# SeanNaren/deepspeech.pytorch

Hardware: NVIDIA H100
Metric: utterances/sec (train step, 161x1000 spectrogram) (higher is better)
Workload: dtype fp16-operands(rnn)+tf32(conv/fc)

## Files before the change

deepspeech.pytorch_b200/csrc/rnn_persistent_tc.cu:

```cuda
#include <cooperative_groups.h>
#include <cuda_fp16.h>
#include <dlfcn.h>
#include <stdlib.h>

#include "common.cuh"
#include "rnn_cells.cuh"
#include "rnn_common.cuh"
#include "tc_common.cuh"

namespace cg = cooperative_groups;

namespace ds2 {

namespace rp {
constexpr int UT = 16;
constexpr int MM = 64;
constexpr int BK = 32;
constexpr int STAGES = 8;
constexpr int THREADS = 288;
constexpr int A_BYTES = MM * 128;
constexpr long long SPIN_LIMIT = 4000000000LL;
}

struct PersistParams {
// ... 475 lines not shown
  int max_clusters = 0;
  if (cudaOccupancyMaxActiveClusters(&max_clusters, kern, &c.cfg) != cudaSuccess) {
    (void)cudaGetLastError();
    return -1;
  }
  return max_clusters * cluster;
}

template <typename Prepare>
static int launch_sweep(SweepKernel kern, int cluster, int per_dir, size_t smem, int fit, bool per_dir_ok,
                        size_t ctl_bytes, const char* what, const char* fallback, PersistParams& p, cudaStream_t st,
                        Prepare&& prepare) {
  int grid = p.D * per_dir, launches = 1;
  if (fit < grid) {
    if (!per_dir_ok || fit < per_dir) return 1;
    grid = per_dir;
    launches = p.D;
  }
  if (int rc = prepare()) return rc;
  DS2_CHECK_CUDA(cudaMemsetAsync(p.err, 0, ctl_bytes, st));
  SweepConfig c(cluster, grid, smem, st);
  for (int li = 0; li < launches; ++li) {
    p.d0 = li;
    if (cluster == 0) {
      void* args[] = {&p};
      DS2_CHECK_CUDA(cudaLaunchCooperativeKernel((const void*)kern, dim3(grid), dim3(rp::THREADS), args, smem, st));
    } else {
      const cudaError_t le = cudaLaunchKernelEx(&c.cfg, kern, p);
      if (le != cudaSuccess) {
        (void)cudaGetLastError();
        if (li == 0) {
          if (fallback)
            fprintf(stderr, "ds2_b200: WARNING %s launch failed (%s); using %s\n", what, cudaGetErrorString(le), fallback);
          return 1;
        }
        set_error("%s: second launch failed: %s", what, cudaGetErrorString(le));
        return DS2_ERR_CUDA;
      }
    }
    g_launches.fetch_add(1, std::memory_order_relaxed);
  }
  DS2_LAUNCH(sweep_check_kernel, 1, 1, 0, st, p.err);
  return DS2_OK;
}

static size_t fwd_smem_bytes(int NB) {
  using namespace rp;
  size_t NBp = NB + 1;
  return 1024 + (size_t)STAGES * (A_BYTES + (size_t)NB * 128) + (5 * UT * NBp + NB + 4) * sizeof(float) +
         (2 * STAGES + 2) * sizeof(uint64_t) + 64 + tc::acc_image_bytes(NB);
}

static size_t splitk_res_ws_bytes(int G, int T, int B, int H, int D);

size_t rnn_sweep_tc_workspace_bytes(int rnn, int T, int B, int H, int D) {
  const int G = rnn == DS2_RNN_LSTM ? 4 : (rnn == DS2_RNN_GRU ? 3 : 1);
  const size_t fwd = 4096 + align_up((size_t)D * G * H * H * 2, 256) + align_up((size_t)D * T * B * H * 2, 256);
  const size_t bwd = splitk_res_ws_bytes(G, T, B, H, D);
  return (fwd > bwd ? fwd : bwd) + 256;
}

static bool fwd_eligible(const SeqArgs& a) {
  if (a.h0 || a.c0) return false;
  if (a.H % 32 != 0 || a.B > 256 || a.T < 2) return false;
  return vec_ok(a.gates, a.hseq, a.aux);
}

__global__ void f32_to_f16_kernel(size_t n, const float* __restrict__ in, __half* __restrict__ out) {
  size_t i = (size_t)blockIdx.x * blockDim.x + threadIdx.x, stride = (size_t)gridDim.x * blockDim.x;
  for (; i < n; i += stride) out[i] = __float2half_rn(in[i]);
}

static size_t res_smem_bytes(int NB, int H) {
  using namespace rp;
  size_t NBp = NB + 1;
  return 1024 + (size_t)(H / 64) * (A_BYTES + (size_t)NB * 128) + (5 * UT * NBp + NB + 4) * sizeof(float) +
         (32 + STAGES + 2) * sizeof(uint64_t) + 64 + tc::acc_image_bytes(NB);
}

static size_t res_ws_bytes(int G, int T, int B, int H, int D) {
  return 4096 + align_up((size_t)D * G * H * H * 2, 256) + align_up((size_t)D * T * B * H * 2, 256);
}

static int f16_weight_maps(const SeqArgs& a, PersistParams& p, void* ws, int chunks, cudaStream_t st) {
  using namespace rp;
  const int G = a.G;
  __half* w16 = reinterpret_cast<__half*>(static_cast<char*>(ws) + 4096);
  p.h16 = reinterpret_cast<__half*>(static_cast<char*>(ws) + 4096 + align_up((size_t)a.D * G * a.H * a.H * 2, 256));
  const size_t wn = (size_t)G * a.H * a.H;
  p.box3 = chunks % 4 == 0;
  for (int d = 0; d < a.D; ++d) {
    DS2_LAUNCH(f32_to_f16_kernel, 132 * 4, 256, 0, st, wn, a.w_hh[d], w16 + (size_t)d * wn);
    int rc = make_tmap_f16(&p.tmW[d], w16 + (size_t)d * wn, 3, a.H, a.H, G, (size_t)a.H, (size_t)a.H * a.H, 64, UT, G);
    if (rc) return rc;
    rc = make_tmap_f16(&p.tmV[d], p.h16 + (size_t)d * a.T * a.B * a.H, 2, a.H, a.T * a.B, 1, (size_t)a.H, 0, 64, a.B, 1);
    if (rc) return rc;
    if (p.box3) {
      rc = make_tmap_f16(&p.tmV3[d], p.h16 + (size_t)d * a.T * a.B * a.H, 3, 64, a.T * a.B, a.H / 64, (size_t)a.H, 64, 64,
                         p.NB, 4);
      if (rc) return rc;
    }
  }
  return DS2_OK;
}

template <int RNN>
static int launch_fwd_resident(const SeqArgs& a, void* ws, size_t ws_bytes, cudaStream_t st) {
  const int G = RNN == DS2_RNN_LSTM ? 4 : (RNN == DS2_RNN_GRU ? 3 : 1);
  if (a.H % 64 != 0 || a.H / 64 > 32) return 1;
  if (!vec_ok(a.gates, a.hseq, a.aux)) return 1;
  if (ws_bytes < res_ws_bytes(G, a.T, a.B, a.H, a.D)) return 1;
  PersistParams p = sweep_params(a, rp::UT, "DS2_TRACE_FWD", ws);
  if (p.NB > 128) return 1;
  const size_t smem = one_cta_per_sm(res_smem_bytes(p.NB, a.H));
  if (smem > 227 * 1024) return 1;
  const SweepKernel kern = rnn_fwd_persist_kernel<RNN, true>;
  static DeviceOnce attr_once;
  int fit = 0;
  if (int rc = opt_in_smem(attr_once, {kern})) return rc;
  if (int rc = coop_fit(kern, smem, &fit)) return rc;
  return launch_sweep(kern, 0, p.NT, smem, fit, true, 4096, nullptr, nullptr, p, st,
                      [&] { return f16_weight_maps(a, p, ws, a.H / 64, st); });
}

template <int RNN>
static int launch_fwd_splitk(const SeqArgs& a, void* ws, size_t ws_bytes, cudaStream_t st);

template <int RNN>
static int launch_fwd(const SeqArgs& a, void* ws, size_t ws_bytes, cudaStream_t st) {
  using namespace rp;
  const int G = RNN == DS2_RNN_LSTM ? 4 : (RNN == DS2_RNN_GRU ? 3 : 1);
  if (!getenv("DS2_NO_RESIDENT")) {
    if (RNN != DS2_RNN_TANH && env_flag("DS2_FWD_SPLITK", 1)) {
      constexpr int R = RNN == DS2_RNN_TANH ? DS2_RNN_LSTM : RNN;
      int rc = launch_fwd_splitk<R>(a, ws, ws_bytes, st);
      if (rc != 1) return rc;
    }
    int rc = launch_fwd_resident<RNN>(a, ws, ws_bytes, st);
    if (rc != 1) return rc;
  }
  PersistParams p = sweep_params(a, UT, "DS2_TRACE_FWD", ws);
  if (p.NB > 128) return 1;
  if (ws_bytes < 4096) return 1;
  const size_t smem = one_cta_per_sm(fwd_smem_bytes(p.NB));
  if (smem > 227 * 1024) return 1;
  const SweepKernel kern = rnn_fwd_persist_kernel<RNN, false>;
  static DeviceOnce attr_once;
  int fit = 0;
  if (int rc = opt_in_smem(attr_once, {kern})) return rc;
  if (int rc = coop_fit(kern, smem, &fit)) return rc;
  return launch_sweep(kern, 0, p.NT, smem, fit, true, 4096, nullptr, nullptr, p, st, [&] {
    for (int d = 0; d < a.D; ++d) {
      int rc = make_tmap_3d(&p.tmW[d], a.w_hh[d], a.H, a.H, G, (size_t)a.H, (size_t)a.H * a.H, BK, UT, G);
      if (rc) return rc;
      rc = make_tmap_2d(&p.tmV[d], a.hseq + (size_t)d * a.T * a.B * a.H, a.T * a.B, a.H, a.H, a.B, BK);
      if (rc) return rc;
    }
    return 0;
  });
}

int rnn_sweep_fwd_tc(int rnn, const SeqArgs& a, void* ws, size_t ws_bytes, cudaStream_t st) {
  if (!fwd_eligible(a)) return 1;
  if (rnn == DS2_RNN_LSTM) return launch_fwd<DS2_RNN_LSTM>(a, ws, ws_bytes, st);
  if (rnn == DS2_RNN_GRU) return launch_fwd<DS2_RNN_GRU>(a, ws, ws_bytes, st);
  return launch_fwd<DS2_RNN_TANH>(a, ws, ws_bytes, st);
}

template <int RNN>
__global__ void __launch_bounds__(rp::THREADS, 1) rnn_bwd_persist_kernel(const __grid_constant__ PersistParams p) {
  using namespace rp;
  using namespace tc;
  constexpr int G = RNN == DS2_RNN_LSTM ? 4 : (RNN == DS2_RNN_GRU ? 3 : 1);
  extern __shared__ uint8_t smem_raw[];
  uint8_t* smem = smem_raw + ((1024u - (tc::smem_u32(smem_raw) & 1023u)) & 1023u);
  const int NB = p.NB, B = p.B, T = p.T, H = p.H, D = p.D;
// ... 607 lines not shown
            __half h[NPF];
#pragma unroll
            for (int j = 0; j < NPF; ++j) {
              h[j] = to_half_sat(o[g][j] * nscale);
              t16[((size_t)g * H + j) * TBs] = h[j];
            }
            const __half2 lo = __halves2half2(h[0], h[1]), hi = __halves2half2(h[2], h[3]);
            uint2 pk;
            pk.x = *reinterpret_cast<const unsigned int*>(&lo);
            pk.y = *reinterpret_cast<const unsigned int*>(&hi);
            *reinterpret_cast<uint2*>(r16 + g * H) = pk;
          }
          if (RNN == DS2_RNN_GRU) {
            __half* a16 = p.auxn16T + ((size_t)d * H + u0 + uq) * TBs + col;
#pragma unroll
            for (int j = 0; j < NPF; ++j) a16[(size_t)j * TBs] = to_half_sat(o[4][j] * nscale);
          }
        }
      };
      const bool defer = RES && p.defer && single;
      float sv[5][NPF];
      if (single) {
        finish4(b_own, kc, pdy, pvalid, sv);
        if (!defer && b_own < B) store_dg(b_own, sv);
      } else {
        for (int b = b_own; b < B; b += 32) {
          load_coefs(b, kc, pdy, pvalid);
          finish4(b, kc, pdy, pvalid, sv);
          store_dg(b, sv);
        }
      }
      if (RES) {
#pragma unroll
        for (int o = 16; o > 0; o >>= 1) lmax = fmaxf(lmax, __shfl_xor_sync(0xffffffffu, lmax, o));
        if (lane == 0) atomicMax(cta_max, __float_as_uint(lmax));
      }
      if (e == 0) trace_stamp(p.trace, p.T, step, 8);
      named_bar_sync(1, 128);
      if (e == 0) {
        trace_stamp(p.trace, p.T, step, 9);
        if (RES) {
          atomicMax(p.gmax + (size_t)d * (T + 1) + step + 1, cta_max[0]);
          cta_max[0] = 0u;
        }
        fence_proxy_async_global();
        trace_stamp(p.trace, p.T, step, 10);
        red_release(ctr, 1u);
        trace_stamp(p.trace, p.T, step, 11);
        trace_stamp_ns(p.trace, p.T, step, 12);
      }
      if (defer) {
        if (b_own < B) store_dg(b_own, sv);
        if (e == 0) trace_stamp(p.trace, p.T, step, 13);
      }
    }
    if (p.dbias[d]) {
      named_bar_sync(1, 128);
      float* red = part;
#pragma unroll
      for (int i = 0; i < 5; ++i) {
#pragma unroll
        for (int j = 0; j < 4; ++j) {
          float v = bsum[i][j];
          v += __shfl_xor_sync(0xffffffffu, v, 4);
          v += __shfl_xor_sync(0xffffffffu, v, 8);
          v += __shfl_xor_sync(0xffffffffu, v, 16);
          if (lane < 4) red[(q * 5 + i) * 16 + 4 * lane + j] = v;
        }
      }
      named_bar_sync(1, 128);
      if (e < 80) {
        const int i = e / 16, u = e % 16;
        const float v = (red[(0 * 5 + i) * 16 + u] + red[(1 * 5 + i) * 16 + u]) +
                        (red[(2 * 5 + i) * 16 + u] + red[(3 * 5 + i) * 16 + u]);
        if (i < G) p.dbias[d][(size_t)i * H + u0 + u] = v;
        else if (RNN == DS2_RNN_GRU && i == 4) p.dbias_hn[d][u0 + u] = v;
      }
    }
  }
  __syncthreads();
  if constexpr (!XG) cluster_sync_all();
}

template <int RNN, int NKR_T = 0>
__global__ void __launch_bounds__(rp::THREADS, 1) rnn_fwd_splitk_kernel(const __grid_constant__ PersistParams p) {
  using namespace rp;
  using namespace tc;
  constexpr int G = RNN == DS2_RNN_LSTM ? 4 : 3;
  constexpr int AW = 128 * 128;
  extern __shared__ uint8_t smem_raw[];
  uint8_t* smem = smem_raw + ((1024u - (tc::smem_u32(smem_raw) & 1023u)) & 1023u);
  const int NB = p.NB, B = p.B, T = p.T, H = p.H, D = p.D;
  const int B_BYTES = NB * 128;
  const int NBp = NB + 1;
  const int NKR = NKR_T ? NKR_T : H / 128;
  const int NG = grp_count(NKR);
  float* part = reinterpret_cast<float*>(smem + NKR * (AW + B_BYTES));
  float* cst = part + 2 * xt_slice(64, NB);
  int* lens_s = reinterpret_cast<int*>(cst + UT * NBp);
  uint64_t* full = reinterpret_cast<uint64_t*>(lens_s + ((NB + 1) & ~1));
  uint64_t* wbar = full + 8;
  uint64_t* accum_bar = wbar + 1;
  uint64_t* part_bar = accum_bar + 1;
  float* acc_img = reinterpret_cast<float*>(part_bar + 1);

  const int warp = threadIdx.x / 32, lane = threadIdx.x % 32;
  const int rank = blockIdx.x & 1, cl = blockIdx.x >> 1;
  const int NTc = H / 32;
  const int d = p.d0 + cl / NTc, U0 = (cl % NTc) * 32;
  const int u0 = U0 + rank * UT;
  const int GH = G * H;
  unsigned int* ctr = p.bar + 32 * d;
  const unsigned int n_arrive = (unsigned int)(NTc * 2);

  if (warp == 0 && lane == 0) {
    tma_prefetch_desc(&p.tmW[d]);
    tma_prefetch_desc(&p.tmV[d]);
    for (int i = 0; i < 8; ++i) mbar_init(&full[i], 1);
    mbar_init(wbar, 1);
    mbar_init(accum_bar, 1);
    mbar_init(part_bar, 1);
    fence_barrier_init();
  }
  for (int i = threadIdx.x; i < UT * NBp; i += THREADS) cst[i] = 0.f;
  for (int i = threadIdx.x; i < NB; i += THREADS) lens_s[i] = i < B ? p.len[i] : 0;
  __syncthreads();
  cluster_sync_all();
  const int kc0 = rank * NKR;

  if (warp == 8) {
    if (lane == 0) {
      mbar_arrive_expect_tx(wbar, (uint32_t)(NKR * 2 * G * UT * 128));
      for (int c = 0; c < NKR; ++c) {
        tma_load_3d(smem + c * AW, &p.tmW[d], wbar, (kc0 + c) * 64, U0, 0);
        tma_load_3d(smem + c * AW + 64 * 128, &p.tmW[d], wbar, (kc0 + c) * 64, U0 + UT, 0);
      }
      uint8_t* hbuf = smem + NKR * AW;
      for (int step = 1; step < T; ++step) {
        const int t = d == 0 ? step : T - 1 - step;
        const int tp = d == 0 ? t - 1 : t + 1;
        grid_wait_counter(ctr, n_arrive * (unsigned int)step, p.err);
        fence_proxy_async_global();
        trace_stamp(p.trace, p.T, step, 0);
        for (int g = 0; g < NG; ++g) {
          uint64_t* fb = full + g;
          const int c0 = grp_begin(g), c1 = min(NKR, grp_begin(g + 1));
          if (p.box3) {
            mbar_arrive_expect_tx(fb, (uint32_t)(4 * B_BYTES));
            tma_load_3d(hbuf + c0 * B_BYTES, &p.tmV3[d], fb, 0, tp * B, kc0 + c0);
          } else {
            mbar_arrive_expect_tx(fb, (uint32_t)((c1 - c0) * B * 128));
            for (int c = c0; c < c1; ++c) tma_load_2d(hbuf + c * B_BYTES, &p.tmV[d], fb, (kc0 + c) * 64, tp * B);
          }
        }
        trace_stamp(p.trace, p.T, step, 1);
      }
    }
  } else if (warp >= 4) {
    with_nch<2>(NB, [&](auto nch) {
      WgAcc<2, decltype(nch)::value> acc;
      {
        const uint64_t a_base = warp_uniform(smem_desc_sw128(smem_u32(smem)));
        const uint64_t b_base = warp_uniform(smem_desc_sw128(smem_u32(smem + NKR * AW)));
        const uint64_t a_step = (uint64_t)(AW >> 4), b_step = (uint64_t)(B_BYTES >> 4);
        mbar_wait(wbar, 0);
        uint32_t ph = 0;
        for (int step = 1; step < T; ++step) {
          if constexpr (NKR_T > 0) {
            constexpr int NGT = (NKR_T + 3) / 4;
  #pragma unroll
            for (int g = 0; g < NGT; ++g) {
              mbar_wait(full + g, ph);
              if (g == 0 && lane == 0) trace_stamp(p.trace, p.T, step, 2);
              if (g == NGT - 1 && lane == 0) trace_stamp(p.trace, p.T, step, 3);
  #pragma unroll
              for (int c = 4 * g; c < (4 * g + 4 < NKR_T ? 4 * g + 4 : NKR_T); ++c) {
                const uint64_t ad = a_base + (uint64_t)c * a_step, bd = b_base + (uint64_t)c * b_step;
                wg_mma4<true>(acc, ad, bd, c > 0);
              }
            }
          } else {
            for (int g = 0; g < NG; ++g) {
              mbar_wait(full + g, ph);
              if (g == 0 && lane == 0) trace_stamp(p.trace, p.T, step, 2);
              const int c0 = grp_begin(g), c1 = min(NKR, grp_begin(g + 1));
              if (c1 == NKR && lane == 0) trace_stamp(p.trace, p.T, step, 3);
              for (int c = c0; c < c1; ++c) {
                const uint64_t ad = a_base + (uint64_t)c * a_step, bd = b_base + (uint64_t)c * b_step;
                wg_mma4<true>(acc, ad, bd, c > 0);
              }
            }
          }
          wg_publish(acc, acc_img, accum_bar);
          if (lane == 0) trace_stamp(p.trace, p.T, step, 4);
          ph ^= 1;
        }
      }
    });
  } else {
    const int q = warp % 4;
    const int e = threadIdx.x;
    const int dst_cta = q >> 1;
    const int my_row = 32 * (q & 1) + lane;
    const uint32_t dst_row = mapa_u32(smem_u32(part), (uint32_t)dst_cta) + (uint32_t)(rank * xt_slice(64, NB) * 4);
    const uint32_t dst_bar = mapa_u32(smem_u32(part_bar), (uint32_t)dst_cta);
    const uint32_t part_tx = (uint32_t)(2 * 64 * NB * 4);
    const int uq = 4 * (e & 3), b_own = e >> 2;
    float bsum[G][4], bhn[4];
#pragma unroll
    for (int j = 0; j < 4; ++j) {
#pragma unroll
      for (int g = 0; g < G; ++g) {
        const float bx = p.b_ih[d][g * H + u0 + uq + j], bh = p.b_hh[d][g * H + u0 + uq + j];
        bsum[g][j] = (RNN == DS2_RNN_GRU && g == 2) ? bx : bx + bh;
        if (RNN == DS2_RNN_GRU && g == 2) bhn[j] = bh;
      }
      if (RNN != DS2_RNN_GRU) bhn[j] = 0.f;
    }
    auto ld4 = [](const float* src, float (&v)[4]) {
      const float4 x = *reinterpret_cast<const float4*>(src);
      v[0] = x.x; v[1] = x.y; v[2] = x.z; v[3] = x.w;
    };
    auto st4 = [](float* dst, const float (&v)[4]) { *reinterpret_cast<float4*>(dst) = make_float4(v[0], v[1], v[2], v[3]); };
    uint32_t acc_phase = 0, part_phase = 0;
    const bool single = B <= 32;
    for (int step = 0; step < T; ++step) {
      const int t = d == 0 ? step : T - 1 - step;
      float gx[G][4];
      if (single && b_own < B) {
#pragma unroll
        for (int g = 0; g < G; ++g) ld4(p.gates + (((size_t)t * B + b_own) * D + d) * GH + (size_t)g * H + u0 + uq, gx[g]);
      }
      if (step > 0) {
        if (e == 0) mbar_arrive_expect_tx(part_bar, part_tx);
        mbar_wait(accum_bar, acc_phase);
        if (e == 0) trace_stamp(p.trace, p.T, step, 5);
        for (int cb = 0; cb < NB; cb += 32) {
          float acc[32];
          tmem_ld32(acc_img, acc_pitch(NB), ((uint32_t)(q * 32) << 16) + (uint32_t)cb, acc);
#pragma unroll
          for (int i = 0; i < 8; ++i) {
            const int c0 = cb + 4 * i;
            if (c0 < NB)
              st_async_v4(dst_row + (uint32_t)(xt_off(64, my_row, c0) * 4), acc[4 * i], acc[4 * i + 1], acc[4 * i + 2], acc[4 * i + 3], dst_bar);
          }
        }
        acc_phase ^= 1;
        if (e == 0) trace_stamp(p.trace, p.T, step, 6);
        mbar_wait_cluster(part_bar, part_phase, p.err);
        part_phase ^= 1;
      }
      if (e == 0) trace_stamp(p.trace, p.T, step, 7);
      auto cell4 = [&](int b, const float (&x)[G][4], float (&o)[6][4]) {
        const bool valid = t < lens_s[b];
        float pre[G][4], hn[4], hval[4];
#pragma unroll
        for (int g = 0; g < G; ++g)
#pragma unroll
          for (int j = 0; j < 4; ++j) {
            float r = 0.f;
            if (step > 0) {
              const float* pr = part + xt_off(64, g * UT + uq + j, b);
              r = pr[0] + pr[xt_slice(64, NB)];
            }
            if (RNN == DS2_RNN_GRU && g == 2) { hn[j] = r + bhn[j]; pre[g][j] = x[g][j] + bsum[g][j]; }
            else pre[g][j] = (x[g][j] + r) + bsum[g][j];
          }
        if (RNN == DS2_RNN_LSTM) {
          float a[4][4], cval[4], th[4];
#pragma unroll
          for (int g = 0; g < 4; ++g)
#pragma unroll
            for (int j = 0; j < 4; ++j) a[g][j] = ex2_ftz((g == 2 ? -2.f * LOG2E : -LOG2E) * pre[g][j]);
#pragma unroll
          for (int g = 0; g < 4; ++g)
#pragma unroll
            for (int j = 0; j < 4; ++j) a[g][j] = rcp_ftz(1.f + a[g][j]);
#pragma unroll
          for (int j = 0; j < 4; ++j) {
            a[2][j] = fmaf(2.f, a[2][j], -1.f);
            cval[j] = valid ? fmaf(a[1][j], cst[(uq + j) * NBp + b], a[0][j] * a[2][j]) : 0.f;
          }
#pragma unroll
          for (int j = 0; j < 4; ++j) th[j] = ex2_ftz(-2.f * LOG2E * cval[j]);
#pragma unroll
          for (int j = 0; j < 4; ++j) th[j] = rcp_ftz(1.f + th[j]);
#pragma unroll
          for (int j = 0; j < 4; ++j) {
            hval[j] = valid ? a[3][j] * fmaf(2.f, th[j], -1.f) : 0.f;
            if (valid) cst[(uq + j) * NBp + b] = cval[j];
#pragma unroll
            for (int g = 0; g < 4; ++g) o[g][j] = valid ? a[g][j] : 0.f;
            o[4][j] = cval[j];
          }
        } else {
          float a[2][4], nv[4];
#pragma unroll
          for (int g = 0; g < 2; ++g)
#pragma unroll
            for (int j = 0; j < 4; ++j) a[g][j] = ex2_ftz(-LOG2E * pre[g][j]);
#pragma unroll
          for (int g = 0; g < 2; ++g)
#pragma unroll
            for (int j = 0; j < 4; ++j) a[g][j] = rcp_ftz(1.f + a[g][j]);
#pragma unroll
          for (int j = 0; j < 4; ++j) nv[j] = ex2_ftz(-2.f * LOG2E * fmaf(a[0][j], hn[j], pre[2][j]));
#pragma unroll
          for (int j = 0; j < 4; ++j) nv[j] = rcp_ftz(1.f + nv[j]);
#pragma unroll
          for (int j = 0; j < 4; ++j) {
            const float nval = valid ? fmaf(2.f, nv[j], -1.f) : 0.f;
            const float hprev = cst[(uq + j) * NBp + b];
            hval[j] = valid ? fmaf(a[1][j], hprev - nval, nval) : 0.f;
            if (valid) cst[(uq + j) * NBp + b] = hval[j];
            o[0][j] = valid ? a[0][j] : 0.f; o[1][j] = valid ? a[1][j] : 0.f; o[2][j] = nval; o[3][j] = 0.f;
            o[4][j] = valid ? hn[j] : 0.f;
          }
        }
#pragma unroll
        for (int j = 0; j < 4; ++j) o[5][j] = hval[j];
        const __half2 lo = __floats2half2_rn(hval[0], hval[1]), hi = __floats2half2_rn(hval[2], hval[3]);
        uint2 pk;
        pk.x = *reinterpret_cast<const unsigned int*>(&lo);
        pk.y = *reinterpret_cast<const unsigned int*>(&hi);
        *reinterpret_cast<uint2*>(p.h16 + (((size_t)d * T + t) * B + b) * H + u0 + uq) = pk;
      };
      auto store4 = [&](int b, const float (&o)[6][4]) {
        const size_t so = (((size_t)d * T + t) * B + b) * H + u0 + uq;
        float* gp = p.gates + (((size_t)t * B + b) * D + d) * GH + u0 + uq;
        st4(p.aux + so, o[4]);
        if (p.training) {
#pragma unroll
          for (int g = 0; g < G; ++g) st4(gp + g * H, o[g]);
        }
        st4(p.hseq + so, o[5]);
      };
      const bool defer = p.defer && single;
      float sv[6][4];
      if (single) {
        if (b_own < B) {
          cell4(b_own, gx, sv);
          if (!defer) store4(b_own, sv);
        }
      } else {
        for (int b = b_own; b < B; b += 32) {
#pragma unroll
          for (int g = 0; g < G; ++g) ld4(p.gates + (((size_t)t * B + b) * D + d) * GH + (size_t)g * H + u0 + uq, gx[g]);
          cell4(b, gx, sv);
          store4(b, sv);
        }
      }
      if (e == 0) trace_stamp(p.trace, p.T, step, 8);
      named_bar_sync(1, 128);
      if (e == 0) {
        trace_stamp(p.trace, p.T, step, 9);
        fence_proxy_async_global();
        trace_stamp(p.trace, p.T, step, 10);
        red_release(ctr, 1u);
        trace_stamp(p.trace, p.T, step, 11);
        trace_stamp_ns(p.trace, p.T, step, 12);
      }
      if (defer) {
        if (b_own < B) store4(b_own, sv);
        if (e == 0) trace_stamp(p.trace, p.T, step, 13);
      }
    }
  }
  __syncthreads();
  cluster_sync_all();
}

static size_t fwd_splitk_smem_bytes(int NB, int H) {
  using namespace rp;
  size_t NBp = NB + 1;
  return 1024 + (size_t)(H / 128) * (128 * 128 + (size_t)NB * 128) + (2 * xt_slice(64, NB) + UT * NBp + NB + 4) * sizeof(float) +
         12 * sizeof(uint64_t) + 64 + tc::acc_image_bytes(NB);
}

template <int RNN>
static int launch_fwd_splitk(const SeqArgs& a, void* ws, size_t ws_bytes, cudaStream_t st) {
  constexpr int G = RNN == DS2_RNN_LSTM ? 4 : 3;
  if (a.H % 128 != 0 || a.H / 128 > 32) return 1;
  if (!vec_ok(a.gates, a.hseq, a.aux) || !a.aux) return 1;
  if (ws_bytes < res_ws_bytes(G, a.T, a.B, a.H, a.D)) return 1;
  PersistParams p = sweep_params(a, 32, "DS2_TRACE_FWD", ws);
  if (p.NB > 64) return 1;
  const size_t smem = one_cta_per_sm(fwd_splitk_smem_bytes(p.NB, a.H));
  if (smem > 227 * 1024) return 1;
  const SweepKernel kern = a.H == 1024 ? rnn_fwd_splitk_kernel<RNN, 8> : rnn_fwd_splitk_kernel<RNN, 0>;
  static DeviceOnce attr_once;
  if (int rc = opt_in_smem(attr_once, {rnn_fwd_splitk_kernel<RNN, 8>, rnn_fwd_splitk_kernel<RNN, 0>})) return rc;
  const int fit = cluster_fit(kern, 2, a.D * p.NT * 2, smem, st);
  return launch_sweep(kern, 2, p.NT * 2, smem, fit, true, 4096, "split-K forward sweep", "the 16-unit kernel", p, st,
                      [&] { return f16_weight_maps(a, p, ws, a.H / 128, st); });
}

static size_t splitk_smem_bytes(int NB, int CL) {
  using namespace rp;
  size_t NBp = NB + 1;
  return 1024 + (size_t)STAGES * ((size_t)UT * CL * 128 + (size_t)NB * 128) +
         ((size_t)CL * xt_slice(UT, NB) + UT * NBp + NB + 16) * sizeof(float) + (2 * STAGES + 3) * sizeof(uint64_t) + 64 + tc::acc_image_bytes(NB);
}

__global__ void absmax_rows_kernel(size_t n, const float* __restrict__ x, unsigned int* __restrict__ out) {
  __shared__ float red[8];
  const float* row = x + (size_t)blockIdx.x * n;
  float m = 0.f;
  for (size_t i = threadIdx.x * 4; i + 3 < n; i += blockDim.x * 4) {
    const float4 v = *reinterpret_cast<const float4*>(row + i);
    m = fmaxf(m, fmaxf(fmaxf(fabsf(v.x), fabsf(v.y)), fmaxf(fabsf(v.z), fabsf(v.w))));
  }
  for (size_t i = (n & ~(size_t)3) + threadIdx.x; i < n; i += blockDim.x) m = fmaxf(m, fabsf(row[i]));
#pragma unroll
  for (int o = 16; o > 0; o >>= 1) m = fmaxf(m, __shfl_xor_sync(0xffffffffu, m, o));
  if (threadIdx.x % 32 == 0) red[threadIdx.x / 32] = m;
  __syncthreads();
  if (threadIdx.x == 0) {
    for (int w = 1; w < (int)(blockDim.x / 32); ++w) m = fmaxf(m, red[w]);
    out[blockIdx.x] = __float_as_uint(m);
  }
}

static size_t splitk_res_smem_bytes(int NB, int Kc, int CL) {
  using namespace rp;
  size_t NBp = NB + 1;
  return 1024 + (size_t)(Kc / 64) * ((size_t)UT * CL * 128 + (size_t)NB * 128) +
         ((size_t)CL * xt_slice(UT, NB) + UT * NBp + NB + 16) * sizeof(float) + (32 + STAGES + 3) * sizeof(uint64_t) + 64 + tc::acc_image_bytes(NB);
}
constexpr size_t XCNT_OFFSET = 1024;
constexpr int XCNT_MAX = (4096 - (int)XCNT_OFFSET) / 4;
static size_t splitk_xbuf_bytes(int B, int H, int D) {
  return (size_t)D * (H / 16) * 4 * 2 * xt_slice(rp::UT, (B + 31) / 32 * 32) * sizeof(float);
}
static size_t splitk_res_ws_bytes(int G, int T, int B, int H, int D) {
  const size_t GH = (size_t)G * H;
  return 4096 + align_up((size_t)D * (T + 1) * 4, 256) + align_up((size_t)T * 4, 256) +
         align_up((size_t)D * H * GH * 2, 256) + align_up((size_t)T * B * D * GH * 2, 256) +
         align_up(splitk_xbuf_bytes(B, H, D), 256);
}

template <int RNN, int CL>
static int launch_bwd_splitk_resident(const SeqArgs& a, void* ws, size_t ws_bytes, cudaStream_t st) {
  using namespace rp;
  const int G = RNN == DS2_RNN_LSTM ? 4 : (RNN == DS2_RNN_GRU ? 3 : 1);
  const int GH = G * a.H;
  constexpr int UM = UT * CL;
  if (a.H % UM != 0 || GH % CL != 0 || (GH / CL) % 64 != 0 || (GH / CL) / 64 > 120) return 1;
  if (CL == 8 && ((a.B + 7) / 8 * 8) % 16 != 0) return 1;
  if (!vec_ok(a.gates, a.hseq, a.aux, a.dy)) return 1;
  if (ws_bytes < splitk_res_ws_bytes(G, a.T, a.B, a.H, a.D)) return 1;
  PersistParams p = sweep_params(a, UM, "DS2_TRACE_BWD", ws);
  if (p.NB > (CL == 8 ? 64 : 128)) return 1;
  for (int d = 0; d < a.D; ++d) { p.dbias[d] = a.dbias[d]; p.dbias_hn[d] = a.dbias_hn[d]; }
  if (a.f16_dg && a.f16_dgT && a.f16_scale && (RNN != DS2_RNN_GRU || a.f16_auxT)) {
    p.dgn16 = static_cast<__half*>(a.f16_dg);
    p.dgn16T = static_cast<__half*>(a.f16_dgT);
    p.auxn16T = static_cast<__half*>(a.f16_auxT);
    p.nscale = a.f16_scale;
  }
  char* base = static_cast<char*>(ws);
  size_t off = 4096;
  p.gmax = reinterpret_cast<unsigned int*>(base + off); off += align_up((size_t)a.D * (a.T + 1) * 4, 256);
  p.dymax = reinterpret_cast<unsigned int*>(base + off); off += align_up((size_t)a.T * 4, 256);
  __half* wT16 = reinterpret_cast<__half*>(base + off); off += align_up((size_t)a.D * a.H * GH * 2, 256);
  p.dg16 = reinterpret_cast<__half*>(base + off); off += align_up((size_t)a.T * a.B * a.D * GH * 2, 256);
  p.xbuf = reinterpret_cast<float*>(base + off);
  p.xcnt = reinterpret_cast<unsigned int*>(base + XCNT_OFFSET);
  const size_t smem = one_cta_per_sm(splitk_res_smem_bytes(p.NB, GH / CL, CL));
  if (smem > 227 * 1024) return 1;
  const char* xe = getenv("DS2_SPLITK_XCHG");
  const bool force_cluster = xe && !strcmp(xe, "cluster"), force_global = xe && !strcmp(xe, "global");
  if (force_global && CL != 4) return 1;
  constexpr int NKU = (G * 1024 / CL) / 64;
  SweepKernel kern = a.H == 1024 ? rnn_bwd_splitk_kernel<RNN, true, CL, NKU> : rnn_bwd_splitk_kernel<RNN, true, CL, 0>;
  static DeviceOnce attr_once;
  int rc;
  if constexpr (CL == 4)
// ... 151 lines not shown
```

Baseline: 610.7.

## Keep split-K forward accumulators in registers and fuse the cell into the MMA warpgroup

Reorders the recurrent weight tensor map to a unit-major layout so each CTA's wgmma output rows line up with the units it owns. The MMA warpgroup then keeps accumulators in registers, exchanges only the partner CTA's half through DSMEM, and transposes values across the quad with shuffles. It evaluates the gate nonlinearities directly, with cell state held in registers, which removes the accumulator-image publish, the separate cell warpgroup and the shared-memory cell-state array. When deferred saves are enabled with NB=32, the idle warps write the training-side gate, aux and hseq outputs from a shared staging buffer. The price is higher register pressure, extra shuffles on the per-step critical path, and new named-barrier handshakes between warpgroups.

```diff
diff --git a/deepspeech.pytorch_b200/csrc/rnn_persistent_tc.cu b/deepspeech.pytorch_b200/csrc/rnn_persistent_tc.cu
--- a/deepspeech.pytorch_b200/csrc/rnn_persistent_tc.cu
+++ b/deepspeech.pytorch_b200/csrc/rnn_persistent_tc.cu
@@ -581,7 +581,8 @@
   return 4096 + align_up((size_t)D * G * H * H * 2, 256) + align_up((size_t)D * T * B * H * 2, 256);
 }
 
-static int f16_weight_maps(const SeqArgs& a, PersistParams& p, void* ws, int chunks, cudaStream_t st) {
+static int f16_weight_maps(const SeqArgs& a, PersistParams& p, void* ws, int chunks, cudaStream_t st,
+                           bool unit_major = false) {
   using namespace rp;
   const int G = a.G;
   __half* w16 = reinterpret_cast<__half*>(static_cast<char*>(ws) + 4096);
@@ -590,7 +591,9 @@
   p.box3 = chunks % 4 == 0;
   for (int d = 0; d < a.D; ++d) {
     DS2_LAUNCH(f32_to_f16_kernel, 132 * 4, 256, 0, st, wn, a.w_hh[d], w16 + (size_t)d * wn);
-    int rc = make_tmap_f16(&p.tmW[d], w16 + (size_t)d * wn, 3, a.H, a.H, G, (size_t)a.H, (size_t)a.H * a.H, 64, UT, G);
+    int rc = unit_major
+                 ? make_tmap_f16(&p.tmW[d], w16 + (size_t)d * wn, 3, a.H, G, a.H, (size_t)a.H * a.H, (size_t)a.H, 64, 4, UT)
+                 : make_tmap_f16(&p.tmW[d], w16 + (size_t)d * wn, 3, a.H, a.H, G, (size_t)a.H, (size_t)a.H * a.H, 64, UT, G);
     if (rc) return rc;
     rc = make_tmap_f16(&p.tmV[d], p.h16 + (size_t)d * a.T * a.B * a.H, 2, a.H, a.T * a.B, 1, (size_t)a.H, 0, 64, a.B, 1);
     if (rc) return rc;
@@ -1364,6 +1367,39 @@
   if constexpr (!XG) cluster_sync_all();
 }
 
+__device__ __forceinline__ int fwd_cell_unit(int tid, int k) { return 4 * (tid >> 5) + ((tid >> 4) & 1) + 2 * (k >> 1); }
+__device__ __forceinline__ int fwd_cell_col(int tid, int k) { return 8 * ((tid >> 2) & 3) + 2 * (tid & 3) + (k & 1); }
+
+__device__ __forceinline__ int fwd_store_col(int tid) { return 8 * ((tid >> 2) & 3) + 2 * (tid & 3) + ((tid >> 4) & 1); }
+__device__ __forceinline__ void fwd_units4(const float (&v)[4], float (&u4)[4]) {
+  const bool ub = (threadIdx.x >> 4) & 1;
+  const float r0 = __shfl_xor_sync(0xffffffffu, ub ? v[0] : v[1], 16);
+  const float r1 = __shfl_xor_sync(0xffffffffu, ub ? v[2] : v[3], 16);
+  u4[0] = ub ? r0 : v[0];
+  u4[1] = ub ? v[1] : r0;
+  u4[2] = ub ? r1 : v[2];
+  u4[3] = ub ? v[3] : r1;
+}
+
+__device__ __forceinline__ void quad_transpose(float (&v)[16]) {
+  const int x = (threadIdx.x >> 2) & 3;
+#pragma unroll
+  for (int bit = 0; bit < 2; ++bit) {
+    const bool hi = (x >> bit) & 1;
+#pragma unroll
+    for (int i = 0; i < 4; ++i) {
+      if (i & (1 << bit)) continue;
+      const int i1 = i | (1 << bit);
+#pragma unroll
+      for (int k = 0; k < 4; ++k) {
+        const float r = __shfl_xor_sync(0xffffffffu, hi ? v[4 * i + k] : v[4 * i1 + k], 4 << bit);
+        if (hi) v[4 * i + k] = r;
+        else v[4 * i1 + k] = r;
+      }
+    }
+  }
+}
+
 template <int RNN, int NKR_T = 0>
 __global__ void __launch_bounds__(rp::THREADS, 1) rnn_fwd_splitk_kernel(const __grid_constant__ PersistParams p) {
   using namespace rp;
@@ -1374,17 +1410,14 @@
   uint8_t* smem = smem_raw + ((1024u - (tc::smem_u32(smem_raw) & 1023u)) & 1023u);
   const int NB = p.NB, B = p.B, T = p.T, H = p.H, D = p.D;
   const int B_BYTES = NB * 128;
-  const int NBp = NB + 1;
   const int NKR = NKR_T ? NKR_T : H / 128;
   const int NG = grp_count(NKR);
-  float* part = reinterpret_cast<float*>(smem + NKR * (AW + B_BYTES));
-  float* cst = part + 2 * xt_slice(64, NB);
-  int* lens_s = reinterpret_cast<int*>(cst + UT * NBp);
-  uint64_t* full = reinterpret_cast<uint64_t*>(lens_s + ((NB + 1) & ~1));
+  float4* part = reinterpret_cast<float4*>(smem + NKR * (AW + B_BYTES));
+  const bool stage_saves = p.defer && NB == 32;
+  float4* stage = part + NB * 16;
+  uint64_t* full = reinterpret_cast<uint64_t*>(stage + (stage_saves ? 6 * 128 : 0));
   uint64_t* wbar = full + 8;
-  uint64_t* accum_bar = wbar + 1;
-  uint64_t* part_bar = accum_bar + 1;
-  float* acc_img = reinterpret_cast<float*>(part_bar + 1);
+  uint64_t* part_bar = wbar + 1;
 
   const int warp = threadIdx.x / 32, lane = threadIdx.x % 32;
   const int rank = blockIdx.x & 1, cl = blockIdx.x >> 1;
@@ -1400,22 +1433,19 @@
     tma_prefetch_desc(&p.tmV[d]);
     for (int i = 0; i < 8; ++i) mbar_init(&full[i], 1);
     mbar_init(wbar, 1);
-    mbar_init(accum_bar, 1);
     mbar_init(part_bar, 1);
     fence_barrier_init();
   }
-  for (int i = threadIdx.x; i < UT * NBp; i += THREADS) cst[i] = 0.f;
-  for (int i = threadIdx.x; i < NB; i += THREADS) lens_s[i] = i < B ? p.len[i] : 0;
   __syncthreads();
   cluster_sync_all();
   const int kc0 = rank * NKR;
 
   if (warp == 8) {
     if (lane == 0) {
-      mbar_arrive_expect_tx(wbar, (uint32_t)(NKR * 2 * G * UT * 128));
+      mbar_arrive_expect_tx(wbar, (uint32_t)(NKR * 2 * 64 * 128));
       for (int c = 0; c < NKR; ++c) {
-        tma_load_3d(smem + c * AW, &p.tmW[d], wbar, (kc0 + c) * 64, U0, 0);
-        tma_load_3d(smem + c * AW + 64 * 128, &p.tmW[d], wbar, (kc0 + c) * 64, U0 + UT, 0);
+        tma_load_3d(smem + c * AW, &p.tmW[d], wbar, (kc0 + c) * 64, 0, u0);
+        tma_load_3d(smem + c * AW + 64 * 128, &p.tmW[d], wbar, (kc0 + c) * 64, 0, U0 + (rank ^ 1) * UT);
       }
       uint8_t* hbuf = smem + NKR * AW;
       for (int step = 1; step < T; ++step) {
@@ -1440,223 +1470,257 @@
     }
   } else if (warp >= 4) {
     with_nch<2>(NB, [&](auto nch) {
-      WgAcc<2, decltype(nch)::value> acc;
-      {
-        const uint64_t a_base = warp_uniform(smem_desc_sw128(smem_u32(smem)));
-        const uint64_t b_base = warp_uniform(smem_desc_sw128(smem_u32(smem + NKR * AW)));
-        const uint64_t a_step = (uint64_t)(AW >> 4), b_step = (uint64_t)(B_BYTES >> 4);
-        mbar_wait(wbar, 0);
-        uint32_t ph = 0;
-        for (int step = 1; step < T; ++step) {
+      constexpr int NCH = decltype(nch)::value;
+      const int tid = threadIdx.x - 128;
+      float bsum[G][2], bhn[2];
+#pragma unroll
+      for (int hh = 0; hh < 2; ++hh) {
+        const int u = u0 + fwd_cell_unit(tid, 2 * hh);
+#pragma unroll
+        for (int g = 0; g < G; ++g) {
+          const float bx = p.b_ih[d][g * H + u], bh = p.b_hh[d][g * H + u];
+          bsum[g][hh] = (RNN == DS2_RNN_GRU && g == 2) ? bx : bx + bh;
+          if (RNN == DS2_RNN_GRU && g == 2) bhn[hh] = bh;
+        }
+        if (RNN != DS2_RNN_GRU) bhn[hh] = 0.f;
+      }
+      float cs[NCH][4];
+#pragma unroll
+      for (int c = 0; c < NCH; ++c)
+#pragma unroll
+        for (int k = 0; k < 4; ++k) cs[c][k] = 0.f;
+      const uint32_t dst_part = mapa_u32(smem_u32(part + tid), (uint32_t)(rank ^ 1));
+      const uint32_t dst_bar = mapa_u32(smem_u32(part_bar), (uint32_t)(rank ^ 1));
+      const uint32_t part_tx = (uint32_t)(64 * NB * 4);
+      const uint64_t a_base = warp_uniform(smem_desc_sw128(smem_u32(smem)));
+      const uint64_t b_base = warp_uniform(smem_desc_sw128(smem_u32(smem + NKR * AW)));
+      const uint64_t a_step = (uint64_t)(AW >> 4), b_step = (uint64_t)(B_BYTES >> 4);
+      const bool defer = stage_saves;
+      mbar_wait(wbar, 0);
+      uint32_t ph = 0, part_phase = 0;
+      for (int step = 0; step < T; ++step) {
+        const int t = d == 0 ? step : T - 1 - step;
+        float gx[NCH][G][4];
+        auto load_gx = [&](int c) {
+#pragma unroll
+          for (int k = 0; k < 4; ++k) {
+            const int b = 32 * c + fwd_cell_col(tid, k);
+            const float* src = p.gates + (((size_t)t * B + b) * D + d) * GH + u0 + fwd_cell_unit(tid, k);
+#pragma unroll
+            for (int g = 0; g < G; ++g) gx[c][g][k] = b < B ? src[(size_t)g * H] : 0.f;
+          }
+        };
+        if (NCH == 1) load_gx(0);
+        float s[NCH][16];
+        if (step > 0) {
+          if (tid == 0) mbar_arrive_expect_tx(part_bar, part_tx);
+          WgAcc<2, NCH> acc;
           if constexpr (NKR_T > 0) {
             constexpr int NGT = (NKR_T + 3) / 4;
-  #pragma unroll
+#pragma unroll
             for (int g = 0; g < NGT; ++g) {
               mbar_wait(full + g, ph);
-              if (g == 0 && lane == 0) trace_stamp(p.trace, p.T, step, 2);
-              if (g == NGT - 1 && lane == 0) trace_stamp(p.trace, p.T, step, 3);
-  #pragma unroll
+              if (g == 0 && tid == 0) trace_stamp(p.trace, p.T, step, 2);
+              if (g == NGT - 1 && tid == 0) trace_stamp(p.trace, p.T, step, 3);
+#pragma unroll
               for (int c = 4 * g; c < (4 * g + 4 < NKR_T ? 4 * g + 4 : NKR_T); ++c) {
                 const uint64_t ad = a_base + (uint64_t)c * a_step, bd = b_base + (uint64_t)c * b_step;
                 wg_mma4<true>(acc, ad, bd, c > 0);
               }
             }
           } else {
-            for (int g = 0; g < NG; ++g) {
-              mbar_wait(full + g, ph);
-              if (g == 0 && lane == 0) trace_stamp(p.trace, p.T, step, 2);
-              const int c0 = grp_begin(g), c1 = min(NKR, grp_begin(g + 1));
-              if (c1 == NKR && lane == 0) trace_stamp(p.trace, p.T, step, 3);
-              for (int c = c0; c < c1; ++c) {
-                const uint64_t ad = a_base + (uint64_t)c * a_step, bd = b_base + (uint64_t)c * b_step;
-                wg_mma4<true>(acc, ad, bd, c > 0);
+            for (int c = 0; c < NKR; ++c) {
+              if (c % 4 == 0) {
+                mbar_wait(full + c / 4, ph);
+                if (c == 0 && tid == 0) trace_stamp(p.trace, p.T, step, 2);
+                if (c + 4 >= NKR && tid == 0) trace_stamp(p.trace, p.T, step, 3);
               }
+              const uint64_t ad = a_base + (uint64_t)c * a_step, bd = b_base + (uint64_t)c * b_step;
+              wg_mma4<true>(acc, ad, bd, c > 0);
             }
           }
-          wg_publish(acc, acc_img, accum_bar);
-          if (lane == 0) trace_stamp(p.trace, p.T, step, 4);
+          wg_commit();
+          wg_wait<0>();
           ph ^= 1;
+          if (tid == 0) trace_stamp(p.trace, p.T, step, 4);
+#pragma unroll
+          for (int c = 0; c < NCH; ++c)
+#pragma unroll
+            for (int j = 0; j < 4; ++j)
+              st_async_v4(dst_part + (uint32_t)((4 * c + j) * 128 * 16), acc.r[1][c][4 * j], acc.r[1][c][4 * j + 1],
+                          acc.r[1][c][4 * j + 2], acc.r[1][c][4 * j + 3], dst_bar);
+          if (tid == 0) trace_stamp(p.trace, p.T, step, 6);
+          mbar_wait_cluster(part_bar, part_phase, p.err);
+          part_phase ^= 1;
+          if (tid == 0) trace_stamp(p.trace, p.T, step, 7);
+#pragma unroll
+          for (int c = 0; c < NCH; ++c) {
+#pragma unroll
+            for (int j = 0; j < 4; ++j) {
+              const float4 pv = part[(4 * c + j) * 128 + tid];
+              s[c][4 * j] = acc.r[0][c][4 * j] + pv.x;
+              s[c][4 * j + 1] = acc.r[0][c][4 * j + 1] + pv.y;
+              s[c][4 * j + 2] = acc.r[0][c][4 * j + 2] + pv.z;
+              s[c][4 * j + 3] = acc.r[0][c][4 * j + 3] + pv.w;
+            }
+            quad_transpose(s[c]);
+          }
+        } else {
+#pragma unroll
+          for (int c = 0; c < NCH; ++c)
+#pragma unroll
+            for (int i = 0; i < 16; ++i) s[c][i] = 0.f;
+        }
+        auto cell4 = [&](int c, const float (&x)[G][4], const float (&r4)[16], float (&cp)[4], float (&o)[6][4]) {
+          float pre[G][4], hn[4], hval[4];
+          bool valid[4];
+#pragma unroll
+          for (int k = 0; k < 4; ++k) {
+            const int b = 32 * c + fwd_cell_col(tid, k);
+            valid[k] = b < B && t < p.len[b];
+          }
+#pragma unroll
+          for (int g = 0; g < G; ++g)
+#pragma unroll
+            for (int k = 0; k < 4; ++k) {
+              const float r = r4[4 * g + k];
+              if (RNN == DS2_RNN_GRU && g == 2) { hn[k] = r + bhn[k >> 1]; pre[g][k] = x[g][k] + bsum[g][k >> 1]; }
+              else pre[g][k] = (x[g][k] + r) + bsum[g][k >> 1];
+            }
+          if (RNN == DS2_RNN_LSTM) {
+            float a[4][4], cval[4], th[4];
+#pragma unroll
+            for (int g = 0; g < 4; ++g)
+#pragma unroll
+              for (int k = 0; k < 4; ++k) a[g][k] = ex2_ftz((g == 2 ? -2.f * LOG2E : -LOG2E) * pre[g][k]);
+#pragma unroll
+            for (int g = 0; g < 4; ++g)
+#pragma unroll
+              for (int k = 0; k < 4; ++k) a[g][k] = rcp_ftz(1.f + a[g][k]);
+#pragma unroll
+            for (int k = 0; k < 4; ++k) {
+              a[2][k] = fmaf(2.f, a[2][k], -1.f);
+              cval[k] = valid[k] ? fmaf(a[1][k], cp[k], a[0][k] * a[2][k]) : 0.f;
+            }
+#pragma unroll
+            for (int k = 0; k < 4; ++k) th[k] = ex2_ftz(-2.f * LOG2E * cval[k]);
+#pragma unroll
+            for (int k = 0; k < 4; ++k) th[k] = rcp_ftz(1.f + th[k]);
+#pragma unroll
+            for (int k = 0; k < 4; ++k) {
+              hval[k] = valid[k] ? a[3][k] * fmaf(2.f, th[k], -1.f) : 0.f;
+              if (valid[k]) cp[k] = cval[k];
+#pragma unroll
+              for (int g = 0; g < 4; ++g) o[g][k] = valid[k] ? a[g][k] : 0.f;
+              o[4][k] = cval[k];
+            }
+          } else {
+            float a[2][4], nv[4];
+#pragma unroll
+            for (int g = 0; g < 2; ++g)
+#pragma unroll
+              for (int k = 0; k < 4; ++k) a[g][k] = ex2_ftz(-LOG2E * pre[g][k]);
+#pragma unroll
+            for (int g = 0; g < 2; ++g)
+#pragma unroll
+              for (int k = 0; k < 4; ++k) a[g][k] = rcp_ftz(1.f + a[g][k]);
+#pragma unroll
+            for (int k = 0; k < 4; ++k) nv[k] = ex2_ftz(-2.f * LOG2E * fmaf(a[0][k], hn[k], pre[2][k]));
+#pragma unroll
+            for (int k = 0; k < 4; ++k) nv[k] = rcp_ftz(1.f + nv[k]);
+#pragma unroll
+            for (int k = 0; k < 4; ++k) {
+              const float nval = valid[k] ? fmaf(2.f, nv[k], -1.f) : 0.f;
+              hval[k] = valid[k] ? fmaf(a[1][k], cp[k] - nval, nval) : 0.f;
+              if (valid[k]) cp[k] = hval[k];
+              o[0][k] = valid[k] ? a[0][k] : 0.f; o[1][k] = valid[k] ? a[1][k] : 0.f; o[2][k] = nval; o[3][k] = 0.f;
+              o[4][k] = valid[k] ? hn[k] : 0.f;
+            }
+          }
+#pragma unroll
+          for (int k = 0; k < 4; ++k) o[5][k] = hval[k];
+        };
+        const int bs = fwd_store_col(tid);
+        const int us = u0 + 4 * (tid >> 5);
+        auto store4 = [&](int c, const float (&o)[6][4]) {
+          const int b = 32 * c + bs;
+          if (b < B) {
+            const size_t so = (((size_t)d * T + t) * B + b) * H + us;
+            float* gp = p.gates + (((size_t)t * B + b) * D + d) * GH + us;
+            *reinterpret_cast<float4*>(p.aux + so) = make_float4(o[4][0], o[4][1], o[4][2], o[4][3]);
+            if (p.training) {
+#pragma unroll
+              for (int g = 0; g < G; ++g)
+                *reinterpret_cast<float4*>(gp + (size_t)g * H) = make_float4(o[g][0], o[g][1], o[g][2], o[g][3]);
+            }
+            *reinterpret_cast<float4*>(p.hseq + so) = make_float4(o[5][0], o[5][1], o[5][2], o[5][3]);
+          }
+        };
+        float sv[NCH][6][4];
+#pragma unroll
+        for (int c = 0; c < NCH; ++c) {
+          if (NCH > 1) load_gx(c);
+          float o[6][4];
+          cell4(c, gx[c], s[c], cs[c], o);
+#pragma unroll
+          for (int q = 0; q < 6; ++q)
+            if (q < G || q >= 4) fwd_units4(o[q], sv[c][q]);
+          const int b = 32 * c + bs;
+          if (b < B) {
+            const __half2 lo = __floats2half2_rn(sv[c][5][0], sv[c][5][1]), hi = __floats2half2_rn(sv[c][5][2], sv[c][5][3]);
+            uint2 pk;
+            pk.x = *reinterpret_cast<const unsigned int*>(&lo);
+            pk.y = *reinterpret_cast<const unsigned int*>(&hi);
+            *reinterpret_cast<uint2*>(p.h16 + (((size_t)d * T + t) * B + b) * H + us) = pk;
+          }
+          if (!defer) store4(c, sv[c]);
+        }
+        if (tid == 0) trace_stamp(p.trace, p.T, step, 8);
+        named_bar_sync(1, 128);
+        if (tid == 0) {
+          trace_stamp(p.trace, p.T, step, 9);
+          fence_proxy_async_global();
+          trace_stamp(p.trace, p.T, step, 10);
+          red_release(ctr, 1u);
+          trace_stamp(p.trace, p.T, step, 11);
+          trace_stamp_ns(p.trace, p.T, step, 12);
+        }
+        if (defer) {
+          named_bar_sync(4, 256);
+#pragma unroll
+          for (int q = 0; q < 6; ++q)
+            if (q < G || q >= 4) stage[q * 128 + tid] = make_float4(sv[0][q][0], sv[0][q][1], sv[0][q][2], sv[0][q][3]);
+          asm volatile("bar.arrive 3, 256;" ::: "memory");
         }
       }
     });
-  } else {
-    const int q = warp % 4;
-    const int e = threadIdx.x;
-    const int dst_cta = q >> 1;
-    const int my_row = 32 * (q & 1) + lane;
-    const uint32_t dst_row = mapa_u32(smem_u32(part), (uint32_t)dst_cta) + (uint32_t)(rank * xt_slice(64, NB) * 4);
-    const uint32_t dst_bar = mapa_u32(smem_u32(part_bar), (uint32_t)dst_cta);
-    const uint32_t part_tx = (uint32_t)(2 * 64 * NB * 4);
-    const int uq = 4 * (e & 3), b_own = e >> 2;
-    float bsum[G][4], bhn[4];
-#pragma unroll
-    for (int j = 0; j < 4; ++j) {
-#pragma unroll
-      for (int g = 0; g < G; ++g) {
-        const float bx = p.b_ih[d][g * H + u0 + uq + j], bh = p.b_hh[d][g * H + u0 + uq + j];
-        bsum[g][j] = (RNN == DS2_RNN_GRU && g == 2) ? bx : bx + bh;
-        if (RNN == DS2_RNN_GRU && g == 2) bhn[j] = bh;
-      }
-      if (RNN != DS2_RNN_GRU) bhn[j] = 0.f;
-    }
-    auto ld4 = [](const float* src, float (&v)[4]) {
-      const float4 x = *reinterpret_cast<const float4*>(src);
-      v[0] = x.x; v[1] = x.y; v[2] = x.z; v[3] = x.w;
-    };
-    auto st4 = [](float* dst, const float (&v)[4]) { *reinterpret_cast<float4*>(dst) = make_float4(v[0], v[1], v[2], v[3]); };
-    uint32_t acc_phase = 0, part_phase = 0;
-    const bool single = B <= 32;
+  } else if (stage_saves) {
+    const int tid = threadIdx.x;
+    const int b = fwd_store_col(tid), us = u0 + 4 * (tid >> 5);
     for (int step = 0; step < T; ++step) {
       const int t = d == 0 ? step : T - 1 - step;
-      float gx[G][4];
-      if (single && b_own < B) {
-#pragma unroll
-        for (int g = 0; g < G; ++g) ld4(p.gates + (((size_t)t * B + b_own) * D + d) * GH + (size_t)g * H + u0 + uq, gx[g]);
-      }
-      if (step > 0) {
-        if (e == 0) mbar_arrive_expect_tx(part_bar, part_tx);
-        mbar_wait(accum_bar, acc_phase);
-        if (e == 0) trace_stamp(p.trace, p.T, step, 5);
-        for (int cb = 0; cb < NB; cb += 32) {
-          float acc[32];
-          tmem_ld32(acc_img, acc_pitch(NB), ((uint32_t)(q * 32) << 16) + (uint32_t)cb, acc);
-#pragma unroll
-          for (int i = 0; i < 8; ++i) {
-            const int c0 = cb + 4 * i;
-            if (c0 < NB)
-              st_async_v4(dst_row + (uint32_t)(xt_off(64, my_row, c0) * 4), acc[4 * i], acc[4 * i + 1], acc[4 * i + 2], acc[4 * i + 3], dst_bar);
-          }
-        }
-        acc_phase ^= 1;
-        if (e == 0) trace_stamp(p.trace, p.T, step, 6);
-        mbar_wait_cluster(part_bar, part_phase, p.err);
-        part_phase ^= 1;
-      }
-      if (e == 0) trace_stamp(p.trace, p.T, step, 7);
-      auto cell4 = [&](int b, const float (&x)[G][4], float (&o)[6][4]) {
-        const bool valid = t < lens_s[b];
-        float pre[G][4], hn[4], hval[4];
-#pragma unroll
-        for (int g = 0; g < G; ++g)
-#pragma unroll
-          for (int j = 0; j < 4; ++j) {
-            float r = 0.f;
-            if (step > 0) {
-              const float* pr = part + xt_off(64, g * UT + uq + j, b);
-              r = pr[0] + pr[xt_slice(64, NB)];
-            }
-            if (RNN == DS2_RNN_GRU && g == 2) { hn[j] = r + bhn[j]; pre[g][j] = x[g][j] + bsum[g][j]; }
-            else pre[g][j] = (x[g][j] + r) + bsum[g][j];
-          }
-        if (RNN == DS2_RNN_LSTM) {
-          float a[4][4], cval[4], th[4];
-#pragma unroll
-          for (int g = 0; g < 4; ++g)
-#pragma unroll
-            for (int j = 0; j < 4; ++j) a[g][j] = ex2_ftz((g == 2 ? -2.f * LOG2E : -LOG2E) * pre[g][j]);
-#pragma unroll
-          for (int g = 0; g < 4; ++g)
-#pragma unroll
-            for (int j = 0; j < 4; ++j) a[g][j] = rcp_ftz(1.f + a[g][j]);
-#pragma unroll
-          for (int j = 0; j < 4; ++j) {
-            a[2][j] = fmaf(2.f, a[2][j], -1.f);
-            cval[j] = valid ? fmaf(a[1][j], cst[(uq + j) * NBp + b], a[0][j] * a[2][j]) : 0.f;
-          }
-#pragma unroll
-          for (int j = 0; j < 4; ++j) th[j] = ex2_ftz(-2.f * LOG2E * cval[j]);
-#pragma unroll
-          for (int j = 0; j < 4; ++j) th[j] = rcp_ftz(1.f + th[j]);
-#pragma unroll
-          for (int j = 0; j < 4; ++j) {
-            hval[j] = valid ? a[3][j] * fmaf(2.f, th[j], -1.f) : 0.f;
-            if (valid) cst[(uq + j) * NBp + b] = cval[j];
-#pragma unroll
-            for (int g = 0; g < 4; ++g) o[g][j] = valid ? a[g][j] : 0.f;
-            o[4][j] = cval[j];
-          }
-        } else {
-          float a[2][4], nv[4];
-#pragma unroll
-          for (int g = 0; g < 2; ++g)
-#pragma unroll
-            for (int j = 0; j < 4; ++j) a[g][j] = ex2_ftz(-LOG2E * pre[g][j]);
-#pragma unroll
-          for (int g = 0; g < 2; ++g)
-#pragma unroll
-            for (int j = 0; j < 4; ++j) a[g][j] = rcp_ftz(1.f + a[g][j]);
-#pragma unroll
-          for (int j = 0; j < 4; ++j) nv[j] = ex2_ftz(-2.f * LOG2E * fmaf(a[0][j], hn[j], pre[2][j]));
-#pragma unroll
-          for (int j = 0; j < 4; ++j) nv[j] = rcp_ftz(1.f + nv[j]);
-#pragma unroll
-          for (int j = 0; j < 4; ++j) {
-            const float nval = valid ? fmaf(2.f, nv[j], -1.f) : 0.f;
-            const float hprev = cst[(uq + j) * NBp + b];
-            hval[j] = valid ? fmaf(a[1][j], hprev - nval, nval) : 0.f;
-            if (valid) cst[(uq + j) * NBp + b] = hval[j];
-            o[0][j] = valid ? a[0][j] : 0.f; o[1][j] = valid ? a[1][j] : 0.f; o[2][j] = nval; o[3][j] = 0.f;
-            o[4][j] = valid ? hn[j] : 0.f;
-          }
-        }
-#pragma unroll
-        for (int j = 0; j < 4; ++j) o[5][j] = hval[j];
-        const __half2 lo = __floats2half2_rn(hval[0], hval[1]), hi = __floats2half2_rn(hval[2], hval[3]);
-        uint2 pk;
-        pk.x = *reinterpret_cast<const unsigned int*>(&lo);
-        pk.y = *reinterpret_cast<const unsigned int*>(&hi);
-        *reinterpret_cast<uint2*>(p.h16 + (((size_t)d * T + t) * B + b) * H + u0 + uq) = pk;
-      };
-      auto store4 = [&](int b, const float (&o)[6][4]) {
-        const size_t so = (((size_t)d * T + t) * B + b) * H + u0 + uq;
-        float* gp = p.gates + (((size_t)t * B + b) * D + d) * GH + u0 + uq;
-        st4(p.aux + so, o[4]);
+      asm volatile("bar.arrive 4, 256;" ::: "memory");
+      named_bar_sync(3, 256);
+      if (b < B) {
+        const size_t so = (((size_t)d * T + t) * B + b) * H + us;
+        float* gp = p.gates + (((size_t)t * B + b) * D + d) * GH + us;
+        *reinterpret_cast<float4*>(p.aux + so) = stage[4 * 128 + tid];
         if (p.training) {
 #pragma unroll
-          for (int g = 0; g < G; ++g) st4(gp + g * H, o[g]);
-        }
-        st4(p.hseq + so, o[5]);
-      };
-      const bool defer = p.defer && single;
-      float sv[6][4];
-      if (single) {
-        if (b_own < B) {
-          cell4(b_own, gx, sv);
-          if (!defer) store4(b_own, sv);
-        }
-      } else {
-        for (int b = b_own; b < B; b += 32) {
-#pragma unroll
-          for (int g = 0; g < G; ++g) ld4(p.gates + (((size_t)t * B + b) * D + d) * GH + (size_t)g * H + u0 + uq, gx[g]);
-          cell4(b, gx, sv);
-          store4(b, sv);
-        }
-      }
-      if (e == 0) trace_stamp(p.trace, p.T, step, 8);
-      named_bar_sync(1, 128);
-      if (e == 0) {
-        trace_stamp(p.trace, p.T, step, 9);
-        fence_proxy_async_global();
-        trace_stamp(p.trace, p.T, step, 10);
-        red_release(ctr, 1u);
-        trace_stamp(p.trace, p.T, step, 11);
-        trace_stamp_ns(p.trace, p.T, step, 12);
-      }
-      if (defer) {
-        if (b_own < B) store4(b_own, sv);
-        if (e == 0) trace_stamp(p.trace, p.T, step, 13);
-      }
+          for (int g = 0; g < G; ++g) *reinterpret_cast<float4*>(gp + (size_t)g * H) = stage[g * 128 + tid];
+        }
+        *reinterpret_cast<float4*>(p.hseq + so) = stage[5 * 128 + tid];
+      }
+      if (tid == 0) trace_stamp(p.trace, p.T, step, 13);
     }
   }
   __syncthreads();
   cluster_sync_all();
 }
 
-static size_t fwd_splitk_smem_bytes(int NB, int H) {
-  using namespace rp;
-  size_t NBp = NB + 1;
-  return 1024 + (size_t)(H / 128) * (128 * 128 + (size_t)NB * 128) + (2 * xt_slice(64, NB) + UT * NBp + NB + 4) * sizeof(float) +
-         12 * sizeof(uint64_t) + 64 + tc::acc_image_bytes(NB);
+static size_t fwd_splitk_smem_bytes(int NB, int H, bool defer) {
+  return 1024 + (size_t)(H / 128) * (128 * 128 + (size_t)NB * 128) + (size_t)64 * NB * sizeof(float) +
+         (defer && NB == 32 ? 6 * 128 * 16 : 0) + 10 * sizeof(uint64_t) + 64;
 }
 
 template <int RNN>
@@ -1667,14 +1731,14 @@
   if (ws_bytes < res_ws_bytes(G, a.T, a.B, a.H, a.D)) return 1;
   PersistParams p = sweep_params(a, 32, "DS2_TRACE_FWD", ws);
   if (p.NB > 64) return 1;
-  const size_t smem = one_cta_per_sm(fwd_splitk_smem_bytes(p.NB, a.H));
+  const size_t smem = one_cta_per_sm(fwd_splitk_smem_bytes(p.NB, a.H, p.defer));
   if (smem > 227 * 1024) return 1;
   const SweepKernel kern = a.H == 1024 ? rnn_fwd_splitk_kernel<RNN, 8> : rnn_fwd_splitk_kernel<RNN, 0>;
   static DeviceOnce attr_once;
   if (int rc = opt_in_smem(attr_once, {rnn_fwd_splitk_kernel<RNN, 8>, rnn_fwd_splitk_kernel<RNN, 0>})) return rc;
   const int fit = cluster_fit(kern, 2, a.D * p.NT * 2, smem, st);
   return launch_sweep(kern, 2, p.NT * 2, smem, fit, true, 4096, "split-K forward sweep", "the 16-unit kernel", p, st,
-                      [&] { return f16_weight_maps(a, p, ws, a.H / 128, st); });
+                      [&] { return f16_weight_maps(a, p, ws, a.H / 128, st, true); });
 }
 
 static size_t splitk_smem_bytes(int NB, int CL) {
```

Measured after the change: 630.4, median of 6. 1.03x the previous value.
